# MatteoMartinelli97/RNNWavefunctions

Hardware: AMD Instinct MI355X
Metric: samples*sites/sec (autoregressive sample+local_energy), 1D TFIM N=80 nh=50 (higher is better)
Workload: dtype f32 (bf16x3 split, f32 accumulate)

## Files before the change

### include/rnnwf.h

```cpp
#ifndef RNNWF_H
#define RNNWF_H

#include <stdint.h>

#ifdef __cplusplus
extern "C" {
#endif

#define RNNWF_ABI_VERSION 1

typedef struct rnnwf_handle rnnwf_handle;

typedef enum {
    RNNWF_OK = 0,
    RNNWF_ERR_INVALID = -1,
    RNNWF_ERR_HIP = -2,
    RNNWF_ERR_STATE = -3,
    RNNWF_ERR_COMM = -4,
    RNNWF_ERR_NOMEM = -5,
    RNNWF_ERR_NUMERIC = -6
} rnnwf_status;

typedef enum {
    RNNWF_MODEL_GRU1D = 0,
// ... 44 lines not shown
int rnnwf_tfim2d_eloc(rnnwf_handle* h, const int32_t* samples, int64_t numsamples, const double* Jz, double Bx,
                      double* eloc, double* log_probs);

int rnnwf_j1j2_eloc(rnnwf_handle* h, const int32_t* samples, int64_t numsamples, const double* J1,
                    const double* J2, const double* Bz, int32_t periodic, int32_t marshall,
                    float* eloc_re_im, int64_t* n_connected);

int rnnwf_vmc_step(rnnwf_handle* h, int64_t numsamples, uint64_t seed, uint64_t step, int64_t sample_offset,
                   const double* couplings, int64_t n_couplings, int32_t* out_samples, void* out_eloc,
                   double* moments);

int rnnwf_vmc_gradient(rnnwf_handle* h, double mean_energy, double mean_energy_im, double norm);
int rnnwf_load_batch(rnnwf_handle* h, const int32_t* samples, int64_t ns, const void* eloc);
int rnnwf_get_grad(rnnwf_handle* h, const char* tf_name, void* data, int64_t count, int32_t dtype);
int rnnwf_set_params_flat(rnnwf_handle* h, const double* flat, int64_t count);
int rnnwf_get_grads_flat(rnnwf_handle* h, double* flat, int64_t count);
const char* rnnwf_param_name(const rnnwf_handle* h, int32_t i, int64_t* count);
int rnnwf_allreduce_grads(rnnwf_handle* h);

int rnnwf_device_training_supported(rnnwf_handle* h);
int rnnwf_adam_step(rnnwf_handle* h, double learning_rate, double beta1, double beta2, double epsilon);
int rnnwf_train_steps(rnnwf_handle* h, int32_t K, int64_t numsamples, uint64_t seed, uint64_t step0, int64_t sample_offset,
                      const double* couplings, int64_t n_couplings, const double* learning_rates, double beta1, double beta2,
                      double epsilon, double* moments);
int rnnwf_adam_get_state(rnnwf_handle* h, double* m_flat, double* v_flat, int64_t count, int64_t* t_steps);
int rnnwf_adam_set_state(rnnwf_handle* h, const double* m_flat, const double* v_flat, int64_t count, int64_t t_steps);

int rnnwf_renyi2_swap(rnnwf_handle* h, const int32_t* samples, int64_t npairs, uint64_t seed, uint64_t step,
                      int64_t pair_offset, double* sums, double* out_log_ratio, int32_t* out_samples);

// ... 99 lines not shown
```

### rnnwavefunctions_amd/_lib.py

```python
import ctypes as C
import os

import numpy as np

_HERE = os.path.dirname(os.path.abspath(__file__))
LIB_PATH = os.path.join(_HERE, "lib", "librnnwf_hip.so")

MODEL_GRU1D, MODEL_GRU1D_PARITY, MODEL_CRNN_U1, MODEL_GRU1D_F64, MODEL_MDRNN2D, MODEL_LSTM1D_F64 = range(6)
F32, F64 = 0, 1
ABI_VERSION = 1
MAX_LAYERS = 4
UNIQUE_ID_BYTES = 128
SR_BLOCK = 32
SR_COMPLEX_MAX_SAMPLES = 2048


class Config(C.Structure):
    _fields_ = [("abi_version", C.c_int32), ("model", C.c_int32), ("nx", C.c_int32), ("ny", C.c_int32),
                ("num_layers", C.c_int32), ("units", C.c_int32 * MAX_LAYERS), ("device", C.c_int32),
                ("reserved", C.c_int32 * 6)]


_P = C.c_void_p
_I32P, _F64P, _F32P = C.POINTER(C.c_int32), C.POINTER(C.c_double), C.POINTER(C.c_float)
# ... 9 lines not shown
    "rnnwf_get_param": (C.c_int, [_P, C.c_char_p, _P, _I64, _I32]),
    "rnnwf_commit_params": (C.c_int, [_P]),
    "rnnwf_init_params": (C.c_int, [_P, C.c_uint64]),
    "rnnwf_num_params": (_I64, [_P]),
    "rnnwf_sample": (C.c_int, [_P, _I64, _U64, _U64, _I64, _I32P, _F64P]),
    "rnnwf_log_prob": (C.c_int, [_P, _I32P, _I64, _F64P]),
    "rnnwf_log_amp": (C.c_int, [_P, _I32P, _I64, _F32P]),
    "rnnwf_tfim_eloc": (C.c_int, [_P, _I32P, _I64, _F64P, _F64, _F64P, _F64P]),
    "rnnwf_tfim2d_eloc": (C.c_int, [_P, _I32P, _I64, _F64P, _F64, _F64P, _F64P]),
    "rnnwf_j1j2_eloc": (C.c_int, [_P, _I32P, _I64, _F64P, _F64P, _F64P, _I32, _I32, _F32P, C.POINTER(_I64)]),
    "rnnwf_vmc_step": (C.c_int, [_P, _I64, _U64, _U64, _I64, _F64P, _I64, _I32P, _P, _F64P]),
    "rnnwf_vmc_gradient": (C.c_int, [_P, _F64, _F64, _F64]),
    "rnnwf_load_batch": (C.c_int, [_P, _I32P, _I64, _P]),
    "rnnwf_get_grad": (C.c_int, [_P, C.c_char_p, _P, _I64, _I32]),
    "rnnwf_set_params_flat": (C.c_int, [_P, _F64P, _I64]),
    "rnnwf_get_grads_flat": (C.c_int, [_P, _F64P, _I64]),
    "rnnwf_param_name": (C.c_char_p, [_P, _I32, C.POINTER(_I64)]),
    "rnnwf_allreduce_grads": (C.c_int, [_P]),
    "rnnwf_comm_unique_id": (C.c_int, [_P]),
    "rnnwf_comm_init": (C.c_int, [_P, _P, _I32, _I32]),
    "rnnwf_allreduce_moments": (C.c_int, [_P, _F64P, _I32]),
    "rnnwf_allreduce_f64": (C.c_int, [_P, _F64P, _I64]),
    "rnnwf_comm_info": (C.c_int, [_P, _P, _P, _P]),
    "rnnwf_comm_reduce_in_step": (C.c_int, [_P, _I32]),
    "rnnwf_comm_destroy": (C.c_int, [_P]),
    "rnnwf_device_training_supported": (C.c_int, [_P]),
    "rnnwf_adam_step": (C.c_int, [_P, _F64, _F64, _F64, _F64]),
    "rnnwf_train_steps": (C.c_int, [_P, _I32, _I64, C.c_uint64, C.c_uint64, _I64, _F64P, _I64, _F64P, _F64, _F64, _F64, _F64P]),
    "rnnwf_adam_get_state": (C.c_int, [_P, _F64P, _F64P, _I64, C.POINTER(_I64)]),
    "rnnwf_adam_set_state": (C.c_int, [_P, _F64P, _F64P, _I64, _I64]),
# ... 730 lines not shown
```

### rnnwavefunctions_amd/csrc/handle.h

```cpp
#pragma once
#include <hip/hip_runtime.h>

#include <algorithm>
#include <cstdarg>
#include <cstring>
#include <cstdio>
#include <map>
#include <string>
#include <type_traits>
#include <utility>
#include <vector>

#include "../../include/rnnwf.h"

namespace rnnwf {

struct Family;

struct DevBuf {
    void* p = nullptr;
    size_t cap = 0;
};

enum TimerId : int { kTimerBase = 0, kTimerFlip = 1, kTimerAssembly = 2, kTimerBackprop = 3, kTimerGemm = 4, kTimerCount };
// ... 62 lines not shown
    std::string err;
    hipStream_t stream = nullptr;
    std::map<std::string, rnnwf::ParamSpec> params;
    std::map<std::string, std::vector<int32_t>> param_flat;
    bool committed = false;

    rnnwf::DevBuf wimg, samples_i32, bits, bits2, hck, lpq, lpq2, out_lp, out_lp2, eloc, moments, coupl, maps;
    rnnwf::DevBuf camp, tiles, tile_count, cbase, cout;
    rnnwf::DevBuf rowbuf;
    rnnwf::DevBuf wbwd, gradP, gradQ, gradW;
    bool wbwd_valid = false;
    rnnwf::DevBuf gradPart, gradHeadPart;
    std::vector<double> coupl_host;
    rnnwf::DevBuf gradDX[2];
    rnnwf::DevBuf wsplit;
    rnnwf::DevBuf wsplit16;
    rnnwf::DevBuf wbasebf;
    rnnwf::DevBuf wsplit_up[RNNWF_MAX_LAYERS - 1];
    rnnwf::DevBuf xrec[2];
    rnnwf::TrainState train;
    bool base_bf = false;
    bool engine_split = false;
    bool engine_forced = false;
    int64_t call_ns = 0;
    int last_flip_engine = -1;
    std::map<std::string, std::vector<double>> grads;
    int64_t last_ns = 0;
    void* pinned = nullptr;
    void* pinned_dev = nullptr;
    double* moments_direct = nullptr;
// ... 215 lines not shown
```

### rnnwavefunctions_amd/csrc/models.h

```cpp
#pragma once
#include <vector>

#include "handle.h"

namespace rnnwf {

int upload_samples(rnnwf_handle* h, const int32_t* samples, int64_t B);
int pack_device(rnnwf_handle* h, int64_t B, DevBuf& bits, int reverse, const int32_t* col_of_pos_dev);
int unpack_device(rnnwf_handle* h, const DevBuf& bits, int64_t B, const int32_t* pos_of_col_dev);
int upload_and_pack(rnnwf_handle* h, const int32_t* samples, int64_t B, DevBuf& bits, int reverse,
                    const int32_t* col_of_pos_dev);
int unpack_and_download(rnnwf_handle* h, const DevBuf& bits, int64_t B, int32_t* out, const int32_t* pos_of_col_dev);
int run_moments(rnnwf_handle* h, const void* eloc_dev, int64_t ns, bool complex_f32, double* moments_host);
int run_tfim_eloc(rnnwf_handle* h, const uint32_t* bits, const double* lpq, int64_t ns, int Nx, int Ny,
                  const int32_t* pos_of_site_dev, const double* Jz_dev, double Bx, double* eloc_dev);
int run_parity_combine(rnnwf_handle* h, const double* a, const double* b, int64_t n, double* out);
int run_parity_share(rnnwf_handle* h, double* lpF, double* lpR, int64_t n);

struct Draw { uint64_t seed, step; int64_t offset; };
struct Gradient;
struct Family {
    const char* name;
    int (*pack_image)(rnnwf_handle* h, std::vector<char>& img);
    int (*pack_table)(rnnwf_handle* h);
// ... 36 lines not shown
    static const char* const names[] = {"GRU1D", "GRU1D_PARITY", "CRNN_U1", "GRU1D_F64", "MDRNN2D", "LSTM1D_F64"};
    return model >= 0 && model < (int)(sizeof names / sizeof *names) ? names[model] : "unknown";
}
int require_gradient(rnnwf_handle* h, const char* what);
int grad_device(rnnwf_handle* h, double mean_energy, double mean_energy_im, double norm, const double* mom_dev, GradImage* im);
int grad_flat_probe(rnnwf_handle* h, std::vector<int32_t>& sidx, GradImage* im);

int crnn_log_amp(rnnwf_handle* h, const int32_t* samples, int64_t B, float* out_re_im, double* out_logp);
int crnn_j1j2_eloc(rnnwf_handle* h, const int32_t* samples, int64_t ns, const double* J1, const double* J2,
                   const double* Bz, int periodic, int marshall, float* eloc, int64_t* ncon);

struct PrnnArgs;
struct CrnnArgs;
int prnn_split_flip(rnnwf_handle* h, const PrnnArgs& a);
double prnn_split_flops_per_step(rnnwf_handle* h);
int prnn_split_pack(rnnwf_handle* h, std::vector<char>& simg);
int prnn_split_flip_stream(rnnwf_handle* h, const PrnnArgs& a, int kt16);
double prnn_split_stream_flops_per_step(rnnwf_handle* h);
int prnn_split_stream_pack(rnnwf_handle* h, std::vector<char>& simg);
int prnn_teacher_base(rnnwf_handle* h, int64_t ns, bool reversed, double* out_lp);
int prnn_plain_base(rnnwf_handle* h, const PrnnArgs& a);
int prnn_stack_base(rnnwf_handle* h, const PrnnArgs& a);
PrnnArgs prnn_base_args(rnnwf_handle* h, int64_t ns);
size_t prnn_hck_bytes_per_block(rnnwf_handle* h);
int lstm_teacher_base(rnnwf_handle* h, int64_t ns);
int crnn_plain_base(rnnwf_handle* h, const CrnnArgs& a);
CrnnArgs crnn_base_args(rnnwf_handle* h, int64_t ns);
size_t crnn_hck_bytes_per_block(rnnwf_handle* h);
int crnn_split_swap_stream(rnnwf_handle* h, const CrnnArgs& a, int64_t max_tiles, int kt16);
double crnn_split_stream_flops_per_step(rnnwf_handle* h);
int crnn_split_stream_pack(rnnwf_handle* h, std::vector<char>& simg);
bool stack_split_available(const rnnwf_handle* h);
size_t stack_record_bytes_per_32_chains(const rnnwf_handle* h, int64_t steps);
template <int NOUT> int stack_pack(rnnwf_handle* h);
int prnn_stack_flip(rnnwf_handle* h, const PrnnArgs& a);
int crnn_stack_swap(rnnwf_handle* h, const CrnnArgs& a, int64_t max_tiles, int64_t max_records);
double stack_split_flops_per_step(rnnwf_handle* h);
int crnn_split_swap(rnnwf_handle* h, const CrnnArgs& a, int64_t max_tiles);
double crnn_split_flops_per_step(rnnwf_handle* h);
int crnn_split_pack(rnnwf_handle* h, std::vector<char>& simg);
bool base_bf_available(const rnnwf_handle* h);
int base_bf_pack(rnnwf_handle* h);
int prnn_base_coop_bf(rnnwf_handle* h, const PrnnArgs& a);
int crnn_base_coop_bf(rnnwf_handle* h, const CrnnArgs& a);
int split_pack_table(rnnwf_handle* h);
int stack_pack_table(rnnwf_handle* h, int layer);
int base_bf_pack_table(rnnwf_handle* h);

struct GradArgs;
using GradKernel = void (*)(GradArgs);
constexpr int kGradWaves = 4;
template <typename T, int NFULL> constexpr bool kGradWide = sizeof(T) == 4 ? NFULL >= 8 : NFULL == 6;
GradKernel grad_wide_kernel(const rnnwf_handle* h);
int grad_bwd_image(rnnwf_handle* h);
int mdrnn_sr_backward(rnnwf_handle* h, double* head_rows);
void train_params_changed_on_host(rnnwf_handle* h);
int train_sync_params_to_host(rnnwf_handle* h);
int train_allreduce_grads_device(rnnwf_handle* h);
int train_prepare(rnnwf_handle* h);
int train_apply_direction(rnnwf_handle* h, const double* col, size_t col_count, double lr, const long long* hold);
// ... 13 lines not shown
```

### rnnwavefunctions_amd/csrc/pack_split.h

```cpp
#pragma once
#include <cmath>
#include <cstring>

#include "pack.h"
#include "split_core.h"
#include "split16_core.h"

namespace rnnwf {

template <int NOUT, class S = double>
std::vector<char> pack_split16_image(const rnnwf_handle* h) {
    using L = S16Layout<NOUT>;
    using Out = PackSink<S>;
    static_assert(NOUT == 1, "the 16x16x32 form carries one head row (positive RNN)");
    const int H = h->H;
    std::vector<char> img(L::BYTES, 0);
    Out::begin(img);
    const std::string pre = kGruPre;
    const auto Wg = pvs<S>(h, pre + "gates/kernel");
    const auto bg = pvs<S>(h, pre + "gates/bias");
    const auto Wci = pvs<S>(h, pre + "candidate/input_projection/kernel");
    const auto bci = pvs<S>(h, pre + "candidate/input_projection/bias");
    const auto Wch = pvs<S>(h, pre + "candidate/hidden_projection/kernel");
    const auto bch = pvs<S>(h, pre + "candidate/hidden_projection/bias");
// ... 217 lines not shown
    float* XC = reinterpret_cast<float*>(img.data() + L::OFF_XC);
    float* WD = reinterpret_cast<float*>(img.data() + L::OFF_WD);
    float* BD = reinterpret_cast<float*>(img.data() + L::OFF_BD);
    for (int hh = 0; hh < 2; ++hh)
        for (int e = 0; e < L::NU; ++e) {
            const int u = L::unit_of(e, hh);
            if (u >= H) continue;
            for (int sgm = 0; sgm < 2; ++sgm)
                Out::put(&XC[(size_t)(sgm * 2 + hh) * L::NUP + e], sc * (bci[u] + Wci[(size_t)sgm * H + u]));
            for (int o = 0; o < NOUT; ++o) Out::put(&WD[((size_t)hh * L::NUP + e) * NOUT + o], head_w(o, u));
        }
    for (int o = 0; o < NOUT; ++o) Out::put(&BD[o], head_b(o));
    return img;
}

template <int NF32, int RJ, int NOUT, class S = double>
std::vector<char> pack_split_upper_image(const rnnwf_handle* h, int layer, bool top) {
    using U = SplitUpperLayout<NF32, RJ, NOUT>;
    using L = typename U::L0;
    using Out = PackSink<S>;
    const int H = h->H;
    std::vector<char> img(U::BYTES, 0);
    Out::begin(img);
    const std::string pre = "multi_rnn_cell/cell_" + std::to_string(layer) + "/cudnn_compatible_gru_cell/";
    const auto Wg = pvs<S>(h, pre + "gates/kernel");
    const auto bg = pvs<S>(h, pre + "gates/bias");
    const auto Wci = pvs<S>(h, pre + "candidate/input_projection/kernel");
    const auto bci = pvs<S>(h, pre + "candidate/input_projection/bias");
    const auto Wch = pvs<S>(h, pre + "candidate/hidden_projection/kernel");
    const auto bch = pvs<S>(h, pre + "candidate/hidden_projection/bias");
// ... 75 lines not shown
```

### rnnwavefunctions_amd/csrc/prnn.hip

```cpp
#include <algorithm>
#include <cstdlib>
#include <type_traits>

#include "gru_kernels.h"
#include "models.h"
#include "pack.h"
#include "shapes.h"

using namespace rnnwf;

namespace {

template <typename T, int NFULL, int NL, int WAVES>
struct Launch {
    using S = GruStack<T, NFULL, NL, 1>;
    using L = GruLayout<T, NFULL, 1>;
    static constexpr bool F32 = std::is_same<T, float>::value;
    static int base(rnnwf_handle* h, const PrnnArgs& a) {
        if constexpr (NL > 1) {
            if constexpr (F32 && MlCoopLayout<NFULL, NL, 1>::FITS && S::SPILL == 0) {
                if (!h->knobs.no_coop) {
                    using ML = MlCoopLayout<NFULL, NL, 1>;
                    return launch_persistent(h, kTimerBase, prnn_base_coop_kernel<NFULL, false, NL>, ML::THREADS, ML::LDS, a.nsb, ML::NB, a);
                }
// ... 166 lines not shown

int64_t max_chains_per_pass(rnnwf_handle* h) {
    size_t per_block = (size_t)(h->NL > 1 ? h->N : std::max(h->N - 1, 1)) * hck_bytes_per_block(h);
    if (h->NL > 1 && h->engine_split)
        per_block += stack_record_bytes_per_32_chains(h, (int64_t)h->N * (h->N - 1) / 2) / 2;
    const int64_t blocks = std::max<int64_t>(1, (int64_t)(state_budget_bytes(h, kDefaultStateBudget) / per_block));
    return blocks * kChains;
}

int pack_image(rnnwf_handle* h, std::vector<char>& img) {
    h->engine_split = !h->f64 && h->knobs.engine != 1 && (h->NL == 1 ? h->NFULL <= 6 : stack_split_available(h));
    h->engine_forced = h->knobs.engine >= 2;
    if (h->engine_split && h->NL > 1) {
        if (int rc = stack_pack<1>(h)) return rc;
    } else if (h->engine_split) {
        std::vector<char> simg;
        if (int rc = prnn_split_pack(h, simg)) return rc;
        if (int rc = ensure(h, h->wsplit, simg.size())) return rc;
        if (int rc = upload(h, h->wsplit.p, simg.data(), simg.size())) return rc;
    }
    if (int rc = base_bf_pack(h)) return rc;
    return with_launch(h, [&](auto k) { img = decltype(k)::pack(h); }) ? 0 : no_kernel(h);
}

int pack_table(rnnwf_handle* h) {
    return with_launch(h, [&](auto k) { decltype(k)::pack_table(h); }) ? 0 : no_kernel(h);
}

}

int rnnwf::prnn_teacher_base(rnnwf_handle* h, int64_t ns, bool reversed, double* out_lp) {
    PrnnArgs a = base_args(h, ns);
    a.bits = (uint32_t*)(reversed ? h->bits2.p : h->bits.p);
    a.hck = h->hck.p;
// ... 24 lines not shown
```

### rnnwavefunctions_amd/csrc/rnnwf_api.hip

```cpp
#include <cstdlib>
#include <algorithm>
#include <cmath>
#include <cstring>

#include "handle.h"
#include "init_params.h"
#include "models.h"
#include "pack.h"
#include "util_kernels.h"

using namespace rnnwf;

static std::string g_create_error;

typedef std::vector<std::pair<int64_t, int64_t>> Segs;
static void declare(rnnwf_handle* h, const std::string& name, std::vector<int64_t> shape, const Segs& rows, const Segs& cols) {
    ParamSpec s;
    s.shape = shape;
    int64_t tr = 0, tc = 0, pr = 0, pc = 0;
    for (auto& g : rows) { tr += g.first; pr += g.second; }
    for (auto& g : cols) { tc += g.first; pc += g.second; }
    s.value.assign((size_t)(pr * pc), 0.0);
    std::vector<int64_t> rmap, cmap;
    { int64_t off = 0; for (auto& g : rows) { for (int64_t i = 0; i < g.first; ++i) rmap.push_back(off + i); off += g.second; } }
// ... 190 lines not shown
}

static void free_buf(DevBuf& b) {
    if (b.p) hipFree(b.p);
    b.p = nullptr;
    b.cap = 0;
}

extern "C" int rnnwf_destroy(rnnwf_handle* h) {
    if (!h) return RNNWF_OK;
    hipSetDevice(h->cfg.device);
    if (h->stream) hipStreamSynchronize(h->stream);
    rnnwf_comm_destroy(h);
    DevBuf* bufs[] = {&h->wimg, &h->samples_i32, &h->bits, &h->bits2, &h->hck, &h->lpq, &h->lpq2, &h->out_lp,
                      &h->out_lp2, &h->eloc, &h->moments, &h->coupl, &h->maps, &h->camp, &h->tiles,
                      &h->tile_count, &h->cbase, &h->cout, &h->rowbuf, &h->wbwd, &h->gradP, &h->gradQ, &h->gradW, &h->gradPart, &h->gradHeadPart, &h->wsplit, &h->wsplit16, &h->wbasebf, &h->gradDX[0], &h->gradDX[1], &h->reduce_scratch, &h->renyi, &h->tck, &h->corr,
                      &h->xrec[0], &h->xrec[1], &h->wsplit_up[0], &h->wsplit_up[1], &h->wsplit_up[2],
                      &h->train.P, &h->train.M, &h->train.V, &h->train.G, &h->train.gidx, &h->train.img[0].table, &h->train.img[1].table,
                      &h->train.img[2].table, &h->train.img[3].table, &h->train.img[4].table, &h->train.img[5].table, &h->train.img[6].table,
                      &h->train.img[7].table, &h->train.combo,
                      &h->srJ, &h->srHead, &h->srMask, &h->srCol, &h->srGram, &h->srY, &h->srFac, &h->srStat};
    static_assert(RNNWF_MAX_LAYERS == 4, "wsplit_up has RNNWF_MAX_LAYERS - 1 entries");
    for (DevBuf* b : bufs) free_buf(*b);
    for (auto& t : h->timers) {
        for (auto& ev : t.pending) { hipEventDestroy(ev.first); hipEventDestroy(ev.second); }
        for (auto& ev : t.pool) { hipEventDestroy(ev.first); hipEventDestroy(ev.second); }
    }
    if (h->pinned) hipHostFree(h->pinned);
    if (h->train.mom_host) hipHostFree(h->train.mom_host);
    if (h->staging) hipHostFree(h->staging);
    if (h->upbuf) hipHostFree(h->upbuf);
// ... 56 lines not shown
}
extern "C" const char* rnnwf_param_name(const rnnwf_handle* h, int32_t i, int64_t* count) {
    if (!h || i < 0) return nullptr;
    for (auto& kv : h->params)
        if (i-- == 0) {
            if (count) *count = (int64_t)kv.second.slot.size();
            return kv.first.c_str();
        }
    return nullptr;
}

extern "C" int64_t rnnwf_num_params(const rnnwf_handle* h) {
    int64_t n = 0;
    if (h) for (auto& kv : h->params) n += (int64_t)kv.second.slot.size();
    return n;
}

extern "C" int rnnwf_init_params(rnnwf_handle* h, uint64_t seed) {
    if (!h) return RNNWF_ERR_INVALID;
    train_params_changed_on_host(h);
    if (seed > 0xffffffffull) return h->fail(RNNWF_ERR_INVALID, "rnnwf_init_params: seed must fit 32 bits (numpy.random.RandomState)");
    NumpyRandomState rng((uint32_t)seed);
    const int64_t H = h->H;
    const bool f32 = !h->f64;
    auto draw = [&](const std::string& name, int64_t rows, int64_t cols, bool vector = false) {
        auto& p = h->params.at(name);
        std::vector<double> tmp;
        glorot_fill(rng, rows, cols, vector, f32, tmp);
        for (size_t i = 0; i < p.slot.size(); ++i) p.value[p.slot[i]] = tmp[i];
        p.set = true;
// ... 391 lines not shown
```

### rnnwavefunctions_amd/csrc/split.hip

```cpp
#include <algorithm>
#include <cstdlib>
#include <type_traits>

#include "crnn_split_kernels.h"
#include "models.h"
#include "pack.h"
#include "pack_split.h"
#include "shapes.h"
#include "split_kernels.h"

using namespace rnnwf;

namespace {

#ifdef RNNWF_DIAGNOSTICS
template <class Launch>
int read_stamps(rnnwf_handle* h, Launch&& launch, size_t waves, int words, std::vector<unsigned long long>& st) {
    unsigned long long* dev = nullptr;
    const size_t bytes = waves * words * sizeof(unsigned long long);
    RNNWF_HIP(h, hipMalloc((void**)&dev, bytes));
    RNNWF_HIP(h, hipMemsetAsync(dev, 0, bytes, h->stream));
    launch(dev);
    RNNWF_HIP(h, hipStreamSynchronize(h->stream));
    st.resize(waves * words);
// ... 18 lines not shown
    return 0;
}
#endif

template <int NF32, int RJ, int WAVES, int MODE>
struct SLaunch {
    using L = SplitLayout<NF32, RJ, 1, MODE>;
    static int flip(rnnwf_handle* h, const PrnnArgs& a, int kt16) {
        if (L::HP > 4 * kt16) return h->fail(RNNWF_ERR_INVALID, "bf16x3 layout wider than the checkpoint rows (%d > %d)", L::HP, 4 * kt16);
        const int64_t ntiles = (int64_t)(a.N - 1) * ((a.ns + 31) / 32);
        return launch_persistent(h, kTimerFlip, prnn_flip_split_kernel<NF32, RJ, WAVES, MODE>, WAVES * 64, L::LDS_BYTES, ntiles, WAVES, a,
                                 h->wsplit.p, kt16);
    }
    static int flip_pp(rnnwf_handle* h, const PrnnArgs& a, int kt16) {
        if constexpr (MODE == 2) {
            const auto kern = prnn_flip_pp_kernel<NF32, RJ>;
            if (L::HP > 4 * kt16) return h->fail(RNNWF_ERR_INVALID, "bf16x3 layout wider than the checkpoint rows (%d > %d)", L::HP, 4 * kt16);
            const int64_t ntiles = (int64_t)(a.N - 1) * ((a.ns + 31) / 32);
            unsigned grid = 0;
            if (int rc = persistent_grid(h, kern, 512, L::BYTES, ntiles, 8, &grid)) return rc;
#ifdef RNNWF_DIAGNOSTICS
            if (getenv("RNNWF_STAMPS")) {
                return read_stamps(h, [&](unsigned long long* buf) { PrnnArgs b = a; b.stamps = buf; kern<<<grid, 512, L::BYTES, h->stream>>>(b, h->wsplit.p, kt16, StackArgs{}); },
                                   (size_t)grid * 8, 16, "RNNWF_STAMPS", grid,
                                   {"mfma_seg", "barrier_after_mfma", "valu_seg_split_part", "barrier_after_valu", "tile_switch", "total_cycles",
                                    "realtime_ticks_100MHz", "iterations", "valu_seg_gates", "valu_seg_head_logsoftmax"});
            }
#endif
            return timed_launch(h, kTimerFlip, kern, grid, 512, L::BYTES, a, h->wsplit.p, kt16, StackArgs{});
        } else {
            return flip(h, a, kt16);
        }
    }
    static std::vector<char> pack(const rnnwf_handle* h) { return pack_split_image<NF32, RJ, 1, MODE>(h); }
    static double mfma_flops_per_step() { return (double)L::NT * L::KS * 32768.0; }
};

template <int NF32, int RJ, int WAVES, int MODE>
struct CSLaunch {
    using L = SplitLayout<NF32, RJ, 3, MODE>;
    static int swap(rnnwf_handle* h, const CrnnArgs& a, int64_t max_tiles, int kt16) {
        return launch_persistent(h, kTimerFlip, crnn_swap_split_kernel<NF32, RJ, WAVES, MODE>, WAVES * 64, L::BYTES, max_tiles, WAVES, a,
                                 h->wsplit.p, kt16);
    }
    static int swap_pp(rnnwf_handle* h, const CrnnArgs& a, int64_t max_tiles, int kt16) {
        if constexpr (MODE == 2) {
            if (L::HP > 4 * kt16) return h->fail(RNNWF_ERR_INVALID, "bf16x3 layout wider than the checkpoint rows (%d > %d)", L::HP, 4 * kt16);
            return launch_persistent(h, kTimerFlip, crnn_swap_pp_kernel<NF32, RJ>, 512, SplitPP<NF32, RJ, 3>::LDS_WITH_SLOTS, max_tiles, 8, a,
                                     h->wsplit.p, kt16, StackArgs{});
// ... 96 lines not shown
}

int rnnwf::base_bf_pack_table(rnnwf_handle* h) {
    return with_bf_base(h, [&](auto b) { pack_base_bf_image<decltype(b)::NF, Lin>(h); }) ? 0 : 1;
}
int rnnwf::split_pack_table(rnnwf_handle* h) {
    const bool cplx = h->model == RNNWF_MODEL_CRNN_U1;
    return with_row(SplitKernels(), h, [&](auto row) {
        using R = decltype(row);
        if (cplx) pack_split_image<R::NF32, R::RJ, 3, R::MODE, Lin>(h);
        else pack_split_image<R::NF32, R::RJ, 1, R::MODE, Lin>(h);
    }) ? 0 : 1;
}

namespace {
constexpr int kStackNF32 = 1, kStackRJ = 9;
using StackL0 = SplitLayout<kStackNF32, kStackRJ, 1, 2>;
using StackU1 = SplitUpperLayout<kStackNF32, kStackRJ, 1>;
using StackU3 = SplitUpperLayout<kStackNF32, kStackRJ, 3>;

}

bool rnnwf::stack_split_available(const rnnwf_handle* h) {
    return !h->f64 && h->NL > 1 && h->NFULL == 3 && h->H <= 50 && h->knobs.engine != 1 &&
           (h->model == RNNWF_MODEL_GRU1D || h->model == RNNWF_MODEL_GRU1D_PARITY || h->model == RNNWF_MODEL_CRNN_U1);
}
size_t rnnwf::stack_record_bytes_per_32_chains(const rnnwf_handle* h, int64_t steps) {
    return (size_t)steps * StackU1::RECORD_FLOATS * 4 * (h->NL > 2 ? 2 : 1);
}
double rnnwf::stack_split_flops_per_step(rnnwf_handle* h) {
// ... 82 lines not shown
int rnnwf::prnn_split_flip(rnnwf_handle* h, const PrnnArgs& a) {
    const int kt16 = 4 * h->NFULL + 1;
    if (riders(h)) return prnn_split_flip_stream(h, a, kt16);
    int rc = 0;
    if (with_layout<SLaunch>(h, [&](auto k) { rc = decltype(k)::flip_pp(h, a, kt16); })) return rc;
    return h->fail(RNNWF_ERR_INVALID, "no bf16x3 kernel for NFULL=%d", h->NFULL);
}
double rnnwf::prnn_split_flops_per_step(rnnwf_handle* h) {
    if (riders(h)) return prnn_split_stream_flops_per_step(h);
    double f = 0;
    with_layout<SLaunch>(h, [&](auto k) { f = decltype(k)::mfma_flops_per_step(); });
    return f;
}


int rnnwf::prnn_split_pack(rnnwf_handle* h, std::vector<char>& simg) {
    if (riders(h)) return prnn_split_stream_pack(h, simg);
    if (with_layout<SLaunch>(h, [&](auto k) { simg = decltype(k)::pack(h); })) return 0;
    return h->fail(RNNWF_ERR_INVALID, "no bf16x3 layout for NFULL=%d", h->NFULL);
}

int rnnwf::crnn_split_swap(rnnwf_handle* h, const CrnnArgs& a, int64_t max_tiles) {
    const int kt16 = 4 * h->NFULL + 1;
    if (riders(h)) return crnn_split_swap_stream(h, a, max_tiles, kt16);
    int rc = 0;
    if (with_layout<CSLaunch>(h, [&](auto k) { rc = decltype(k)::swap_pp(h, a, max_tiles, kt16); })) return rc;
    return h->fail(RNNWF_ERR_INVALID, "no bf16x3 cRNN kernel for NFULL=%d", h->NFULL);
}
double rnnwf::crnn_split_flops_per_step(rnnwf_handle* h) {
    if (riders(h)) return crnn_split_stream_flops_per_step(h);
    double f = 0;
    with_layout<CSLaunch>(h, [&](auto k) { f = decltype(k)::mfma_flops_per_step(); });
    return f;
// ... 9 lines not shown
```

### rnnwavefunctions_amd/csrc/split_kernels.h

```cpp
#pragma once
#include "gru_kernels.h"
#include "split_core.h"
#include "split_pp.h"
#include "pp_kernels.h"
#include "split_riders16_asm.h"

namespace rnnwf {

template <int NF32, int RJ, int WAVES, int MODE>
__global__ void __launch_bounds__(WAVES * 64) prnn_flip_split_kernel(PrnnArgs a, const void* wsplit, int kt16) {
    using C = SplitCore<NF32, RJ, 1, MODE>;
    using L = typename C::L;
    constexpr int NU = C::NU, NR = C::NR;
    extern __shared__ __attribute__((aligned(16))) char lds[];
    C::stage(lds, wsplit);
    const int lane = threadIdx.x & 63, c = lane & 31, hh = lane >> 5;
    const int64_t gw = (int64_t)blockIdx.x * WAVES + (threadIdx.x >> 6);
    const int64_t nw = (int64_t)gridDim.x * WAVES;
    const int N = a.N;
    const int64_t nsb32 = (a.ns + 31) / 32;
    const int64_t ntiles = (int64_t)(N - 1) * nsb32;
    const float* hck = reinterpret_cast<const float*>(a.hck);
    for (int64_t tile = gw; tile < ntiles; tile += nw) {
        const int i = (int)(tile / nsb32);
// ... 139 lines not shown
                d += __shfl_xor(d, 32);
                float lp0, lp1;
                log_softmax2(d + bd0, lp0, lp1);
                lp[X] += (double)(sig_in[X] ? lp1 : lp0);
            }
        }
        if (g == 0) {
            const int64_t row = a.row_of_pos ? a.row_of_pos[i] : i + 1;
#pragma unroll
            for (int X = 0; X < 2; ++X)
                if (valid[X]) a.lpq[row * a.ns + s[X]] += lp[X];
        }
    }
}

template <int NF32, int RJ, bool STACK = false>
__global__ void __launch_bounds__(512) prnn_flip_pp_kernel(PrnnArgs a, const void* wsplit, int kt16, StackArgs st) {
    using PP = SplitPP<NF32, RJ, 1>;
    using C = typename PP::C;
    using L = typename C::L;
    constexpr int NU = C::NU, NT = C::NT, NB = PP::NB;
    extern __shared__ __attribute__((aligned(16))) char lds[];
    __shared__ int max_steps;
    if (threadIdx.x == 0) max_steps = 0;
    C::stage(lds, wsplit);
    const int lane = threadIdx.x & 63, c = lane & 31, hh = lane >> 5;
    const int wave = __builtin_amdgcn_readfirstlane(threadIdx.x >> 6);
    const bool late = wave >= 4;
    const int N = a.N;
    const int64_t nsb32 = (a.ns + 31) / 32;
    const PPWalk walk(wave, (int64_t)(N - 1) * nsb32);
    const float* hck = reinterpret_cast<const float*>(a.hck);
    const int iters = walk.lockstep_iters(&max_steps, [&](int64_t t) { return N - 1 - (int)(t / nsb32); });
// ... 19 lines not shown
        const float* src = checkpoint_src(hck, in, a.nsb, scn, STACK ? st.kstride : kt16, STACK ? st.koff : 0);
#pragma unroll
        for (int e = 0; e < NU; ++e) hn[e] = *checkpoint_entry<L>(src, hh, e);
        const int w = in >> 5;
        wn0 = a.bits[(int64_t)w * a.ns + scn];
        wn1 = (w + 1) * 32 < N ? a.bits[(int64_t)(w + 1) * a.ns + scn] : 0u;
    };
    int64_t rec = 0;
    auto begin_tile = [&]() {
        i = (int)(tile / nsb32);
        const int64_t sb = tile - (int64_t)i * nsb32;
        s = (int)sb * 32 + c;
        valid = s < a.ns;
        sc = valid ? s : (int)a.ns - 1;
#pragma unroll
        for (int e = 0; e < NU; ++e) h[e] = hn[e];
        word = wn0;
        word_next = wn1;
        sig_in = 1 - (int)((word >> (i & 31)) & 1);
        n = i + 1;
        if ((n & 31) == 0) { word = word_next; word_next = load_word((n >> 5) + 1); }
        lp = 0.0;
        if constexpr (STACK) rec = flip_record_start(N, nsb32, i, sb);
    };
    if (active) {
        fetch_tile(tile);
        begin_tile();
        PP::preload(lds, sig_in, lane, acc);
        PP::split(h, B);
    }
    PPStamps stamps(a.stamps);
// ... 200 lines not shown
```

### rnnwavefunctions_amd/csrc/split_pp.h

```cpp
#pragma once
#include "split_core.h"
#include "split_mfma_asm.h"

namespace rnnwf {

#define RNNWF_STAGE() __builtin_amdgcn_sched_barrier(0)

template <int NF32, int RJ, int NOUT>
struct SplitPP {
    using C = SplitCore<NF32, RJ, NOUT, 2>;
    using L = typename C::L;
    static constexpr int NT = C::NT, NU = C::NU, NUA = C::NUA, NQ = C::NQ;
    static constexpr int NB = 3 * NQ + 1;
    static constexpr size_t LDS_WITH_SLOTS = ((L::BYTES + 15) / 16) * 16 + 8 * (size_t)NU * 256;
    static constexpr int NP = NUA / 2;
    using Asm = MfmaSegAsm<NT, NQ>;
    static_assert(Asm::kAvailable, "no hand-scheduled MFMA segment generated for this layout (tools/gen_split_mfma_asm.py)");
    static_assert(NP == 4 * NQ, "mode 2: the aligned units fill whole quads");

    static __device__ __forceinline__ unsigned lds_address(const void* p) {
        return (unsigned)(uintptr_t)(const __attribute__((address_space(3))) char*)p;
    }

    static __device__ __forceinline__ void preload(const char* lds, int sig, int lane, f32x16 (&acc)[NT]) {
// ... 75 lines not shown
            au = acc[3 * (e / 16) + 1][e % 16];
            ac = acc[3 * (e / 16) + 2][e % 16];
        } else {
            const int j = e - 16 * NF32;
            ar = acc[3 * NF32 + (j) / 16][(j) % 16];
            au = acc[3 * NF32 + (RJ + j) / 16][(RJ + j) % 16];
            ac = acc[3 * NF32 + (2 * RJ + j) / 16][(2 * RJ + j) % 16];
        }
    }

    static __device__ __forceinline__ void head_lagged(const f32x16 (&acc)[NT], float (&z)[NOUT]) {
#pragma unroll
        for (int o = 0; o < NOUT; ++o) z[o] = acc[3 * NF32 + (L::HEAD_SLOT + o) / 16][(L::HEAD_SLOT + o) % 16];
    }

    template <int E0, int E1>
    static __device__ __forceinline__ void gate_batch(const f32x16 (&acc)[NT], const float* xcp, float (&h)[NU]) {
        constexpr int n = E1 - E0;
        float ar[n], au[n], ac[n], xc[n];
#pragma unroll
        for (int j = 0; j < n; ++j) xc[j] = xcp[E0 + j];
#pragma unroll
        for (int j = 0; j < n; ++j) slots(acc, E0 + j, ar[j], au[j], ac[j]);
        RNNWF_STAGE();
#pragma unroll
        for (int j = 0; j < n; ++j) { ar[j] = __builtin_amdgcn_exp2f(ar[j]); au[j] = __builtin_amdgcn_exp2f(au[j]); }
        RNNWF_STAGE();
#pragma unroll
        for (int j = 0; j < n; ++j) { ar[j] = 1.0f + ar[j]; au[j] = 1.0f + au[j]; }
        RNNWF_STAGE();
#pragma unroll
        for (int j = 0; j < n; ++j) { ar[j] = __builtin_amdgcn_rcpf(ar[j]); au[j] = __builtin_amdgcn_rcpf(au[j]); }
        RNNWF_STAGE();
#pragma unroll
        for (int j = 0; j < n; ++j) ac[j] = fmaf(ar[j], ac[j], xc[j]);
        RNNWF_STAGE();
#pragma unroll
        for (int j = 0; j < n; ++j) ac[j] = __builtin_amdgcn_exp2f(ac[j]);
        RNNWF_STAGE();
#pragma unroll
        for (int j = 0; j < n; ++j) ac[j] = 1.0f + ac[j];
        RNNWF_STAGE();
#pragma unroll
        for (int j = 0; j < n; ++j) ac[j] = __builtin_amdgcn_rcpf(ac[j]);
        RNNWF_STAGE();
#pragma unroll
        for (int j = 0; j < n; ++j) ac[j] = fmaf(2.0f, ac[j], -1.0f);
        RNNWF_STAGE();
#pragma unroll
        for (int j = 0; j < n; ++j) ar[j] = h[E0 + j] - ac[j];
        RNNWF_STAGE();
#pragma unroll
        for (int j = 0; j < n; ++j) asm("v_fma_f32 %0, %1, %2, %3" : "=v"(h[E0 + j]) : "v"(au[j]), "v"(ar[j]), "v"(ac[j]));
        RNNWF_STAGE();
    }

    static __device__ __forceinline__ void gates(const char* lds, int sig, const f32x16 (&acc)[NT], float (&h)[NU], int lane) {
        const float* xcp = reinterpret_cast<const float*>(lds + L::OFF_XC) + (size_t)((sig * 2 + (lane >> 5)) * L::NUP);
        constexpr int HALF = (NU + 1) / 2;
        gate_batch<0, HALF>(acc, xcp, h);
        gate_batch<HALF, NU>(acc, xcp, h);
    }

// ... 154 lines not shown
```

### rnnwavefunctions_amd/csrc/train.hip

```cpp
#include <cmath>

#include "models.h"
#include "pack.h"
#include "pack_split.h"

using namespace rnnwf;

namespace {

constexpr int kMaxSteps = kTrainMaxSteps;

__device__ __forceinline__ void repack_entry(const PackEntry& t, const double* __restrict__ P, char* __restrict__ img) {
#pragma clang fp contract(off)
    double v = P[t.a];
    if (t.b >= 0) v = (t.kind & PACK_MINUS) ? __dsub_rn(v, P[t.b]) : __dadd_rn(v, P[t.b]);
    if (t.d >= 0) v = __dadd_rn(v, P[t.d]);
    if (t.c != 1.0) v = __dmul_rn(t.c, v);
    const int kind = t.kind & 255;
    if (kind == PACK_F32) {
        *reinterpret_cast<float*>(img + t.off) = (float)v;
    } else if (kind == PACK_F64) {
        *reinterpret_cast<double*>(img + t.off) = v;
    } else {
        float r = (float)v;
// ... 198 lines not shown

int launch_repack(rnnwf_handle* h) {
    TrainState& t = h->train;
    if (int rc = ensure_combo(h)) return rc;
    RepackPlan plan{};
    plan.nimg = t.nimg;
    for (int i = 0; i < t.nimg; ++i) {
        plan.start[i + 1] = plan.start[i] + t.img[i].n;
        plan.target[i] = (char*)t.img[i].target->p;
    }
    if (const int64_t total = plan.start[t.nimg]) {
        repack_all_kernel<<<(unsigned)((total + 255) / 256), 256, 0, h->stream>>>((const PackEntry*)t.combo.p, plan, (const double*)t.P.p);
        RNNWF_HIP(h, hipGetLastError());
    }
    t.dev_newer = true;
    return 0;
}

double adam_lr_t(double lr, double b1, double b2, int64_t t) {
    return lr * std::sqrt(1.0 - std::pow(b2, (double)t)) / (1.0 - std::pow(b1, (double)t));
}

}

int rnnwf::train_allreduce_grads_device(rnnwf_handle* h) {
    TrainState& t = h->train;
    if (!h->comm || !h->gradW.p) return 0;
    if (!t.built) { if (build(h) != 0) { h->err.clear(); return 0; } }
    if (!t.supported) return 0;
    const unsigned blocks = (unsigned)((t.nparams + 255) / 256);
    if (t.dw_f64) grad_flat_kernel<double><<<blocks, 256, 0, h->stream>>>((const int32_t*)t.gidx.p, t.nparams, (const double*)h->gradW.p, (double*)t.G.p);
// ... 155 lines not shown
```

Baseline: 305.4 million.

## Run the ping-pong flip kernel in a rescaled g-state with refolded weights

The GRU hidden state is carried as g = (h+1)/2 inside the K-packed ping-pong flip kernel. Weights, input biases and head weights/biases are refolded into a separate image so the math stays equivalent, which removes the per-gate fma that maps the sigmoid-based tanh back to [-1,1]. A host packer, a device refold kernel run after training repacks, and a new API entry point keep the two images in sync. The cost is an extra weight buffer and refold pass, plus small bf16 rounding differences, because the doubled bf16 weights and the subtracted bias sums are quantised differently.

```diff
diff --git a/include/rnnwf.h b/include/rnnwf.h
--- a/include/rnnwf.h
+++ b/include/rnnwf.h
@@ -82,6 +82,7 @@
 int rnnwf_load_batch(rnnwf_handle* h, const int32_t* samples, int64_t ns, const void* eloc);
 int rnnwf_get_grad(rnnwf_handle* h, const char* tf_name, void* data, int64_t count, int32_t dtype);
 int rnnwf_set_params_flat(rnnwf_handle* h, const double* flat, int64_t count);
+int rnnwf_host_split_images(int32_t units, const double* flat, int64_t count, void* img_h, void* img_g, int64_t cap, int32_t* layout);
 int rnnwf_get_grads_flat(rnnwf_handle* h, double* flat, int64_t count);
 const char* rnnwf_param_name(const rnnwf_handle* h, int32_t i, int64_t* count);
 int rnnwf_allreduce_grads(rnnwf_handle* h);
diff --git a/rnnwavefunctions_amd/_lib.py b/rnnwavefunctions_amd/_lib.py
--- a/rnnwavefunctions_amd/_lib.py
+++ b/rnnwavefunctions_amd/_lib.py
@@ -47,6 +47,7 @@
     "rnnwf_load_batch": (C.c_int, [_P, _I32P, _I64, _P]),
     "rnnwf_get_grad": (C.c_int, [_P, C.c_char_p, _P, _I64, _I32]),
     "rnnwf_set_params_flat": (C.c_int, [_P, _F64P, _I64]),
+    "rnnwf_host_split_images": (C.c_int, [C.c_int32, _F64P, _I64, _P, _P, _I64, _I32P]),
     "rnnwf_get_grads_flat": (C.c_int, [_P, _F64P, _I64]),
     "rnnwf_param_name": (C.c_char_p, [_P, _I32, C.POINTER(_I64)]),
     "rnnwf_allreduce_grads": (C.c_int, [_P]),
diff --git a/rnnwavefunctions_amd/csrc/handle.h b/rnnwavefunctions_amd/csrc/handle.h
--- a/rnnwavefunctions_amd/csrc/handle.h
+++ b/rnnwavefunctions_amd/csrc/handle.h
@@ -100,6 +100,7 @@
     std::vector<double> coupl_host;
     rnnwf::DevBuf gradDX[2];
     rnnwf::DevBuf wsplit;
+    rnnwf::DevBuf wsplit_g;
     rnnwf::DevBuf wsplit16;
     rnnwf::DevBuf wbasebf;
     rnnwf::DevBuf wsplit_up[RNNWF_MAX_LAYERS - 1];
diff --git a/rnnwavefunctions_amd/csrc/models.h b/rnnwavefunctions_amd/csrc/models.h
--- a/rnnwavefunctions_amd/csrc/models.h
+++ b/rnnwavefunctions_amd/csrc/models.h
@@ -74,7 +74,7 @@
 struct CrnnArgs;
 int prnn_split_flip(rnnwf_handle* h, const PrnnArgs& a);
 double prnn_split_flops_per_step(rnnwf_handle* h);
-int prnn_split_pack(rnnwf_handle* h, std::vector<char>& simg);
+int prnn_split_pack(rnnwf_handle* h, std::vector<char>& simg, std::vector<char>& simg_g);
 int prnn_split_flip_stream(rnnwf_handle* h, const PrnnArgs& a, int kt16);
 double prnn_split_stream_flops_per_step(rnnwf_handle* h);
 int prnn_split_stream_pack(rnnwf_handle* h, std::vector<char>& simg);
@@ -104,6 +104,8 @@
 int prnn_base_coop_bf(rnnwf_handle* h, const PrnnArgs& a);
 int crnn_base_coop_bf(rnnwf_handle* h, const CrnnArgs& a);
 int split_pack_table(rnnwf_handle* h);
+bool prnn_split_gstate_layout(const rnnwf_handle* h, int32_t* layout10);
+int split_gstate_refold(rnnwf_handle* h);
 int stack_pack_table(rnnwf_handle* h, int layer);
 int base_bf_pack_table(rnnwf_handle* h);
 
diff --git a/rnnwavefunctions_amd/csrc/pack_split.h b/rnnwavefunctions_amd/csrc/pack_split.h
--- a/rnnwavefunctions_amd/csrc/pack_split.h
+++ b/rnnwavefunctions_amd/csrc/pack_split.h
@@ -255,6 +255,65 @@
     return img;
 }
 
+struct GstateLayout {
+    int NT, NQ, NUP, NOUT;
+    uint32_t OFF_ASP, OFF_CI, OFF_XC, OFF_WD, OFF_BD, BYTES;
+};
+template <class L>
+constexpr GstateLayout gstate_layout() {
+    static_assert(L::MODE == 2 && L::OFF_A == 0, "the g-state form exists for the K-packed layout of the ping-pong kernels");
+    return {L::NT, L::NQ, L::NUP, L::NOUT, (uint32_t)L::OFF_ASP, (uint32_t)L::OFF_CI, (uint32_t)L::OFF_XC, (uint32_t)L::OFF_WD, (uint32_t)L::OFF_BD,
+            (uint32_t)L::BYTES};
+}
+__host__ __device__ inline float gstate_bf16(uint16_t b) {
+    union { uint32_t u; float f; } x;
+    x.u = (uint32_t)b << 16;
+    return x.f;
+}
+__host__ __device__ inline uint32_t gstate_bits(float f) {
+    union { uint32_t u; float f; } x;
+    x.f = f;
+    return x.u;
+}
+__host__ __device__ inline uint32_t gstate_word(const GstateLayout& g, const char* img, uint32_t w) {
+    const uint32_t off = 4 * w, in = reinterpret_cast<const uint32_t*>(img)[w];
+    const uint16_t* A = reinterpret_cast<const uint16_t*>(img);
+    if (off < g.OFF_CI) {
+        const float lo = gstate_bf16((uint16_t)(in & 0xffffu)), hi = gstate_bf16((uint16_t)(in >> 16));
+        return (gstate_bits(lo + lo) >> 16) | (gstate_bits(hi + hi) & 0xffff0000u);
+    }
+    if (off < g.OFF_XC) {
+        const int i = (int)((off - g.OFF_CI) / 4), rho = i & 15, hh_row = (i >> 4) & 1, T = (i >> 5) % g.NT;
+        const int r32 = (rho & 3) | (hh_row << 2) | ((rho >> 2) << 3);
+        double sum = 0.0;
+        for (int hhk = 0; hhk < 2; ++hhk) {
+            const int lane = 32 * hhk + r32;
+            for (int x = 0; x < g.NQ; ++x)
+                for (int jj = 0; jj < 8; ++jj) {
+                    float wv = 0.0f;
+                    for (int a = 2; a >= 0; --a) wv += gstate_bf16(A[((((size_t)T * 3 + a) * g.NQ + x) * 64 + lane) * 8 + jj]);
+                    sum += (double)wv;
+                }
+            const uint16_t* sp = A + g.OFF_ASP / 2 + ((size_t)T * 64 + lane) * 8;
+            sum += (double)((gstate_bf16(sp[5]) + gstate_bf16(sp[3])) + gstate_bf16(sp[0]));
+        }
+        return gstate_bits((float)((double)reinterpret_cast<const float*>(img)[w] - sum));
+    }
+    if (off < g.OFF_WD) return in;
+    const float* WD = reinterpret_cast<const float*>(img + g.OFF_WD);
+    if (off < g.OFF_BD) { const float v = reinterpret_cast<const float*>(img)[w]; return gstate_bits(v + v); }
+    const int o = (int)((off - g.OFF_BD) / 4);
+    if (o >= g.NOUT) return in;
+    double sum = 0.0;
+    for (int e = 0; e < 2 * g.NUP; ++e) sum += (double)WD[(size_t)e * g.NOUT + o];
+    return gstate_bits((float)((double)reinterpret_cast<const float*>(img)[w] - sum));
+}
+inline std::vector<char> gstate_image(const GstateLayout& g, const std::vector<char>& img) {
+    std::vector<char> out(img.size());
+    for (uint32_t w = 0; w < g.BYTES / 4; ++w) reinterpret_cast<uint32_t*>(out.data())[w] = gstate_word(g, img.data(), w);
+    return out;
+}
+
 template <int NF32, int RJ, int NOUT, class S = double>
 std::vector<char> pack_split_upper_image(const rnnwf_handle* h, int layer, bool top) {
     using U = SplitUpperLayout<NF32, RJ, NOUT>;
diff --git a/rnnwavefunctions_amd/csrc/prnn.hip b/rnnwavefunctions_amd/csrc/prnn.hip
--- a/rnnwavefunctions_amd/csrc/prnn.hip
+++ b/rnnwavefunctions_amd/csrc/prnn.hip
@@ -204,10 +204,14 @@
     if (h->engine_split && h->NL > 1) {
         if (int rc = stack_pack<1>(h)) return rc;
     } else if (h->engine_split) {
-        std::vector<char> simg;
-        if (int rc = prnn_split_pack(h, simg)) return rc;
+        std::vector<char> simg, simg_g;
+        if (int rc = prnn_split_pack(h, simg, simg_g)) return rc;
         if (int rc = ensure(h, h->wsplit, simg.size())) return rc;
         if (int rc = upload(h, h->wsplit.p, simg.data(), simg.size())) return rc;
+        if (!simg_g.empty()) {
+            if (int rc = ensure(h, h->wsplit_g, simg_g.size())) return rc;
+            if (int rc = upload(h, h->wsplit_g.p, simg_g.data(), simg_g.size())) return rc;
+        }
     }
     if (int rc = base_bf_pack(h)) return rc;
     return with_launch(h, [&](auto k) { img = decltype(k)::pack(h); }) ? 0 : no_kernel(h);
diff --git a/rnnwavefunctions_amd/csrc/rnnwf_api.hip b/rnnwavefunctions_amd/csrc/rnnwf_api.hip
--- a/rnnwavefunctions_amd/csrc/rnnwf_api.hip
+++ b/rnnwavefunctions_amd/csrc/rnnwf_api.hip
@@ -228,7 +228,7 @@
     rnnwf_comm_destroy(h);
     DevBuf* bufs[] = {&h->wimg, &h->samples_i32, &h->bits, &h->bits2, &h->hck, &h->lpq, &h->lpq2, &h->out_lp,
                       &h->out_lp2, &h->eloc, &h->moments, &h->coupl, &h->maps, &h->camp, &h->tiles,
-                      &h->tile_count, &h->cbase, &h->cout, &h->rowbuf, &h->wbwd, &h->gradP, &h->gradQ, &h->gradW, &h->gradPart, &h->gradHeadPart, &h->wsplit, &h->wsplit16, &h->wbasebf, &h->gradDX[0], &h->gradDX[1], &h->reduce_scratch, &h->renyi, &h->tck, &h->corr,
+                      &h->tile_count, &h->cbase, &h->cout, &h->rowbuf, &h->wbwd, &h->gradP, &h->gradQ, &h->gradW, &h->gradPart, &h->gradHeadPart, &h->wsplit, &h->wsplit_g, &h->wsplit16, &h->wbasebf, &h->gradDX[0], &h->gradDX[1], &h->reduce_scratch, &h->renyi, &h->tck, &h->corr,
                       &h->xrec[0], &h->xrec[1], &h->wsplit_up[0], &h->wsplit_up[1], &h->wsplit_up[2],
                       &h->train.P, &h->train.M, &h->train.V, &h->train.G, &h->train.gidx, &h->train.img[0].table, &h->train.img[1].table,
                       &h->train.img[2].table, &h->train.img[3].table, &h->train.img[4].table, &h->train.img[5].table, &h->train.img[6].table,
@@ -315,6 +315,38 @@
     int64_t n = 0;
     if (h) for (auto& kv : h->params) n += (int64_t)kv.second.slot.size();
     return n;
+}
+
+extern "C" int rnnwf_host_split_images(int32_t units, const double* flat, int64_t count, void* img_h, void* img_g, int64_t cap, int32_t* layout) {
+    auto bad = [&](const std::string& m) {
+        g_create_error = "rnnwf_host_split_images: " + m;
+        return (int)RNNWF_ERR_INVALID;
+    };
+    if (!flat || !img_h || !img_g || !layout || units < 1) return bad("null or empty argument");
+    rnnwf_handle h;
+    h.cfg.model = h.model = RNNWF_MODEL_GRU1D;
+    h.cfg.nx = h.Nx = h.N = 2;
+    h.cfg.num_layers = 1;
+    h.cfg.units[0] = h.H = units;
+    h.family = gru_family();
+    h.NFULL = pick_nfull(units, false, false);
+    if (h.NFULL < 0) return bad("num_units too large");
+    declare_params(&h);
+    if (count != rnnwf_num_params(&h)) return bad("the model has " + std::to_string(rnnwf_num_params(&h)) + " parameters");
+    int64_t off = 0;
+    for (auto& kv : h.params) {
+        ParamSpec& p = kv.second;
+        for (size_t i = 0; i < p.slot.size(); ++i) p.value[p.slot[i]] = flat[off + (int64_t)i];
+        off += (int64_t)p.slot.size();
+        p.set = true;
+    }
+    std::vector<char> a, g;
+    if (prnn_split_pack(&h, a, g) != 0) return bad(h.err);
+    if (g.empty() || !prnn_split_gstate_layout(&h, layout)) return bad("this width has no g-state image (37..50 units)");
+    if ((int64_t)a.size() > cap) return bad("images of " + std::to_string(a.size()) + " bytes");
+    memcpy(img_h, a.data(), a.size());
+    memcpy(img_g, g.data(), g.size());
+    return RNNWF_OK;
 }
 
 extern "C" int rnnwf_init_params(rnnwf_handle* h, uint64_t seed) {
diff --git a/rnnwavefunctions_amd/csrc/split.hip b/rnnwavefunctions_amd/csrc/split.hip
--- a/rnnwavefunctions_amd/csrc/split.hip
+++ b/rnnwavefunctions_amd/csrc/split.hip
@@ -1,5 +1,6 @@
 #include <algorithm>
 #include <cstdlib>
+#include <cstring>
 #include <type_traits>
 
 #include "crnn_split_kernels.h"
@@ -56,25 +57,30 @@
     }
     static int flip_pp(rnnwf_handle* h, const PrnnArgs& a, int kt16) {
         if constexpr (MODE == 2) {
-            const auto kern = prnn_flip_pp_kernel<NF32, RJ>;
+            const auto kern = prnn_flip_pp_kernel<NF32, RJ, false, true>;
+            const void* img = h->wsplit_g.p;
             if (L::HP > 4 * kt16) return h->fail(RNNWF_ERR_INVALID, "bf16x3 layout wider than the checkpoint rows (%d > %d)", L::HP, 4 * kt16);
             const int64_t ntiles = (int64_t)(a.N - 1) * ((a.ns + 31) / 32);
             unsigned grid = 0;
             if (int rc = persistent_grid(h, kern, 512, L::BYTES, ntiles, 8, &grid)) return rc;
 #ifdef RNNWF_DIAGNOSTICS
             if (getenv("RNNWF_STAMPS")) {
-                return read_stamps(h, [&](unsigned long long* buf) { PrnnArgs b = a; b.stamps = buf; kern<<<grid, 512, L::BYTES, h->stream>>>(b, h->wsplit.p, kt16, StackArgs{}); },
+                return read_stamps(h, [&](unsigned long long* buf) { PrnnArgs b = a; b.stamps = buf; kern<<<grid, 512, L::BYTES, h->stream>>>(b, img, kt16, StackArgs{}); },
                                    (size_t)grid * 8, 16, "RNNWF_STAMPS", grid,
                                    {"mfma_seg", "barrier_after_mfma", "valu_seg_split_part", "barrier_after_valu", "tile_switch", "total_cycles",
                                     "realtime_ticks_100MHz", "iterations", "valu_seg_gates", "valu_seg_head_logsoftmax"});
             }
 #endif
-            return timed_launch(h, kTimerFlip, kern, grid, 512, L::BYTES, a, h->wsplit.p, kt16, StackArgs{});
+            return timed_launch(h, kTimerFlip, kern, grid, 512, L::BYTES, a, img, kt16, StackArgs{});
         } else {
             return flip(h, a, kt16);
         }
     }
     static std::vector<char> pack(const rnnwf_handle* h) { return pack_split_image<NF32, RJ, 1, MODE>(h); }
+    static bool gstate(GstateLayout* g) {
+        if constexpr (MODE == 2) { *g = gstate_layout<L>(); return true; }
+        else return false;
+    }
     static double mfma_flops_per_step() { return (double)L::NT * L::KS * 32768.0; }
 };
 
@@ -201,6 +207,33 @@
 }
 
 namespace {
+__global__ void gstate_refold_kernel(GstateLayout g, const char* __restrict__ img, uint32_t* __restrict__ out) {
+    const uint32_t w = blockIdx.x * blockDim.x + threadIdx.x;
+    if (w < g.BYTES / 4) out[w] = gstate_word(g, img, w);
+}
+}
+static bool gstate_of(const rnnwf_handle* h, GstateLayout* g) {
+    bool has = false;
+    if (h->model != RNNWF_MODEL_CRNN_U1 && h->NL == 1 && !riders(h)) with_layout<SLaunch>(h, [&](auto k) { has = decltype(k)::gstate(g); });
+    return has;
+}
+bool rnnwf::prnn_split_gstate_layout(const rnnwf_handle* h, int32_t* layout10) {
+    GstateLayout g{};
+    static_assert(sizeof(GstateLayout) == 40, "ten 32-bit fields");
+    if (!gstate_of(h, &g)) return false;
+    memcpy(layout10, &g, sizeof g);
+    return true;
+}
+int rnnwf::split_gstate_refold(rnnwf_handle* h) {
+    GstateLayout g{};
+    if (!h->wsplit_g.p || !gstate_of(h, &g)) return 0;
+    if (g.BYTES > h->wsplit.cap || g.BYTES > h->wsplit_g.cap) return h->fail(RNNWF_ERR_STATE, "g-state image larger than its buffers");
+    gstate_refold_kernel<<<(g.BYTES / 4 + 255) / 256, 256, 0, h->stream>>>(g, (const char*)h->wsplit.p, (uint32_t*)h->wsplit_g.p);
+    RNNWF_HIP(h, hipGetLastError());
+    return 0;
+}
+
+namespace {
 constexpr int kStackNF32 = 1, kStackRJ = 9;
 using StackL0 = SplitLayout<kStackNF32, kStackRJ, 1, 2>;
 using StackU1 = SplitUpperLayout<kStackNF32, kStackRJ, 1>;
@@ -313,9 +346,14 @@
 }
 
 
-int rnnwf::prnn_split_pack(rnnwf_handle* h, std::vector<char>& simg) {
+int rnnwf::prnn_split_pack(rnnwf_handle* h, std::vector<char>& simg, std::vector<char>& simg_g) {
+    simg_g.clear();
     if (riders(h)) return prnn_split_stream_pack(h, simg);
-    if (with_layout<SLaunch>(h, [&](auto k) { simg = decltype(k)::pack(h); })) return 0;
+    if (with_layout<SLaunch>(h, [&](auto k) {
+            simg = decltype(k)::pack(h);
+            GstateLayout g;
+            if (decltype(k)::gstate(&g)) simg_g = gstate_image(g, simg);
+        })) return 0;
     return h->fail(RNNWF_ERR_INVALID, "no bf16x3 layout for NFULL=%d", h->NFULL);
 }
 
diff --git a/rnnwavefunctions_amd/csrc/split_kernels.h b/rnnwavefunctions_amd/csrc/split_kernels.h
--- a/rnnwavefunctions_amd/csrc/split_kernels.h
+++ b/rnnwavefunctions_amd/csrc/split_kernels.h
@@ -177,9 +177,10 @@
     }
 }
 
-template <int NF32, int RJ, bool STACK = false>
+template <int NF32, int RJ, bool STACK = false, bool GSTATE = false>
 __global__ void __launch_bounds__(512) prnn_flip_pp_kernel(PrnnArgs a, const void* wsplit, int kt16, StackArgs st) {
-    using PP = SplitPP<NF32, RJ, 1>;
+    static_assert(!(STACK && GSTATE), "the layer pipeline's records are h");
+    using PP = SplitPP<NF32, RJ, 1, GSTATE>;
     using C = typename PP::C;
     using L = typename C::L;
     constexpr int NU = C::NU, NT = C::NT, NB = PP::NB;
@@ -229,7 +230,7 @@
         valid = s < a.ns;
         sc = valid ? s : (int)a.ns - 1;
 #pragma unroll
-        for (int e = 0; e < NU; ++e) h[e] = hn[e];
+        for (int e = 0; e < NU; ++e) h[e] = PP::enter(hn[e]);
         word = wn0;
         word_next = wn1;
         sig_in = 1 - (int)((word >> (i & 31)) & 1);
diff --git a/rnnwavefunctions_amd/csrc/split_pp.h b/rnnwavefunctions_amd/csrc/split_pp.h
--- a/rnnwavefunctions_amd/csrc/split_pp.h
+++ b/rnnwavefunctions_amd/csrc/split_pp.h
@@ -6,7 +6,7 @@
 
 #define RNNWF_STAGE() __builtin_amdgcn_sched_barrier(0)
 
-template <int NF32, int RJ, int NOUT>
+template <int NF32, int RJ, int NOUT, bool GSTATE = false>
 struct SplitPP {
     using C = SplitCore<NF32, RJ, NOUT, 2>;
     using L = typename C::L;
@@ -113,6 +113,8 @@
         for (int o = 0; o < NOUT; ++o) z[o] = acc[3 * NF32 + (L::HEAD_SLOT + o) / 16][(L::HEAD_SLOT + o) % 16];
     }
 
+    static __device__ __forceinline__ float enter(float hck) { return GSTATE ? fmaf(0.5f, hck, 0.5f) : hck; }
+
     template <int E0, int E1>
     static __device__ __forceinline__ void gate_batch(const f32x16 (&acc)[NT], const float* xcp, float (&h)[NU]) {
         constexpr int n = E1 - E0;
@@ -143,9 +145,11 @@
 #pragma unroll
         for (int j = 0; j < n; ++j) ac[j] = __builtin_amdgcn_rcpf(ac[j]);
         RNNWF_STAGE();
-#pragma unroll
-        for (int j = 0; j < n; ++j) ac[j] = fmaf(2.0f, ac[j], -1.0f);
-        RNNWF_STAGE();
+        if constexpr (!GSTATE) {
+#pragma unroll
+            for (int j = 0; j < n; ++j) ac[j] = fmaf(2.0f, ac[j], -1.0f);
+            RNNWF_STAGE();
+        }
 #pragma unroll
         for (int j = 0; j < n; ++j) ar[j] = h[E0 + j] - ac[j];
         RNNWF_STAGE();
diff --git a/rnnwavefunctions_amd/csrc/train.hip b/rnnwavefunctions_amd/csrc/train.hip
--- a/rnnwavefunctions_amd/csrc/train.hip
+++ b/rnnwavefunctions_amd/csrc/train.hip
@@ -236,7 +236,7 @@
         RNNWF_HIP(h, hipGetLastError());
     }
     t.dev_newer = true;
-    return 0;
+    return split_gstate_refold(h);
 }
 
 double adam_lr_t(double lr, double b1, double b2, int64_t t) {
```

After: 313.4 million, median of 6. 2.6% higher.
